# uc-vision/smart-tree

Hardware: AMD Instinct MI355X
Metric: points/sec end-to-end (voxelize->sparse-UNet->skeleton), 1M-pt tree (higher is better)
Workload: dtype f32

## Files before the change

### include/smarttree_hip.h

```cpp
#ifndef SMARTTREE_HIP_H
#define SMARTTREE_HIP_H

#include <stdint.h>

#ifdef __cplusplus
extern "C" {
#endif

int st_version(void);
#define ST_BRICK_NEED_COUNTS 4
#define ST_SKELETON_STATS_ENTRIES 16
#define ST_SKELETON_TUNING_ENTRIES 24
int st_abi_entries(int what);
const char* st_last_error(void);
int64_t st_query_workspace(int op, int64_t a, int64_t b, int64_t c);

int64_t st_scan_workspace_bytes(int64_t n);
int st_scan_u32(const uint32_t* in, uint32_t* out, int64_t n, uint32_t* total, void* ws, int64_t ws_bytes, void* stream);
int64_t st_sort_workspace_bytes(int64_t n);
int st_sort_pairs_u32(uint32_t* keys, uint32_t* vals, int64_t n, int key_bits, void* ws, int64_t ws_bytes, void* stream);

int64_t st_voxelize_workspace_bytes(int64_t n_points, int max_blocks, int64_t max_voxels);
int st_voxelize_blocks(const float* xyz, const float* rgb, int64_t n, double voxel_size, double block_size,
                       double buffer_size, int min_points, int max_blocks, int64_t max_voxels, float* feats,
                       int32_t* coords, uint8_t* mask, int64_t* point_index, float* block_centres,
                       int64_t* n_voxels_host, int64_t* n_blocks_host, void* ws, int64_t ws_bytes, void* stream);

int64_t st_hash_capacity(int64_t n);
int st_build_coord_hash(const int32_t* coords, int64_t n, unsigned long long* keys, unsigned* vals, int64_t cap, void* stream);
int st_build_subm_rulebook(const int32_t* coords, int64_t n, const unsigned long long* keys, const unsigned* vals,
                           int64_t cap, int32_t* nbr , void* stream);
int64_t st_spatial_order_workspace_bytes(int64_t n);
int st_spatial_order(const int32_t* coords, int64_t n, int32_t* order , void* ws, int64_t ws_bytes, void* stream);
int st_move_rows(const void* src, int row_words, const int32_t* order, int64_t n, void* dst, int scatter, void* stream);
int st_move_rows_list(const void* src, int row_words, const int32_t* order, const int32_t* list, int64_t n, void* dst, int scatter,
                      void* stream);
int64_t st_strided_workspace_bytes(int64_t n_fine);
int st_build_strided_outputs(const int32_t* coords, int64_t n, int64_t max_out, int32_t* out_coords,
                             unsigned long long* ckeys, unsigned* cvals, int64_t ccap, int64_t* n_out_host,
                             int32_t* extent_host , void* ws, int64_t ws_bytes, void* stream);
int st_build_strided_rulebook(const int32_t* coords, int64_t n, const unsigned long long* fkeys, const unsigned* fvals,
                              int64_t fcap, const int32_t* out_coords, int64_t n_out, const unsigned long long* ckeys,
                              const unsigned* cvals, int64_t ccap, const int32_t* extent_host,
                              int32_t* nbr_down , int32_t* nbr_up ,
                              int32_t* up_order ,
                              void* stream);

int st_sparse_conv_fwd(const float* x0, int c0, const float* x1, int cin, const int32_t* nbr, int K, int64_t n_out,
                       const float* w, int cout, const float* scale, const float* shift, const float* residual,
                       int relu, float* y, const int32_t* row_order ,
                       void* stream, int64_t nbr_stride );
int st_sparse_conv_mfma_fwd(const float* x0, int c0, const float* x1, int cin, const int32_t* nbr, int K, int64_t n_out,
                            const float* wp, int cout, const float* scale, const float* shift, const float* residual,
                            int relu, float* y, const int32_t* row_order ,
                            void* stream, int64_t nbr_stride ,
                            int variant );
int st_sparse_conv_b3_fwd(const float* x0, int c0, const float* x1, int cin, const int32_t* nbr, int K, int64_t n_out, const void* wq,
                          int cout, const float* scale, const float* shift, const float* residual, int relu, float* y,
                          const int32_t* row_order, void* stream, int64_t nbr_stride, int variant);
int st_sparse_conv_f16_fwd(const void* x0, int c0, const void* x1, int cin, const int32_t* nbr, int K, int64_t n_out,
                           const void* w, int cout, const float* scale, const float* shift, const void* residual, int relu,
                           void* y, int in_half, int out_half, const int32_t* row_order, void* stream, int64_t nbr_stride );
int st_sparse_conv_mfma_list_fwd(const float* x0, int c0, const float* x1, int cin, const int32_t* nbr, int K, int64_t n_out,
                                 const float* wp, int cout, const float* scale, const float* shift, const float* residual, int relu,
                                 float* y, const int32_t* row_order, void* stream, int64_t nbr_stride, int variant, int64_t level_rows,
                                 int parity);
int st_sparse_conv_b3_list_fwd(const float* x0, int c0, const float* x1, int cin, const int32_t* nbr, int K, int64_t n_out, const void* wq,
                               int cout, const float* scale, const float* shift, const float* residual, int relu, float* y,
                               const int32_t* row_order, void* stream, int64_t nbr_stride, int variant, int64_t level_rows, int parity);
int st_sparse_conv_f16_list_fwd(const void* x0, int c0, const void* x1, int cin, const int32_t* nbr, int K, int64_t n_out,
                                const void* w, int cout, const float* scale, const float* shift, const void* residual, int relu,
                                void* y, int in_half, int out_half, const int32_t* row_order, void* stream, int64_t nbr_stride,
                                int64_t level_rows, int parity);

int64_t st_brick_pyramid_workspace_bytes(int64_t n0, int n_blocks, int coord_bound, int depth, const int64_t* caps);
int st_brick_pyramid(const int32_t* coords0 , int64_t n0, int n_blocks ,
                     int coord_bound , int depth, const int32_t* blk_seg ,
                     int nseg, const int64_t* caps ,
                     int32_t* order0 , int32_t* const* coords_out ,
                     int32_t* const* subm , int32_t* const* down ,
                     int32_t* const* up , int32_t* const* up_order ,
                     int64_t* counts_host , void* ws, int64_t ws_bytes, void* stream);
int st_brick_pyramid_need(const int32_t* coords0, int64_t n0, int n_blocks, int coord_bound, int depth, const int32_t* blk_seg, int nseg,
                          const int64_t* caps, int32_t* order0, int32_t* const* coords_out, int32_t* const* subm, int32_t* const* down,
                          int32_t* const* up, int32_t* const* up_order, int64_t* counts_host, const unsigned char* inner ,
                          int32_t* const* need_order , int32_t* const* up_need ,
                          int64_t* need_counts_host , void* ws, int64_t ws_bytes, void* stream);
int st_head_param_floats(void);
int st_pointwise_mlp_heads(const float* x, int64_t n, const float* params, float* radius, float* direction,
                           float* class_l, float* medial_vector , int64_t* class_idx , void* stream);
int st_pointwise_mlp_heads_keep(const float* x, int64_t n, const unsigned char* keep, const float* params, float* radius, float* direction,
                                float* class_l, float* medial_vector , int64_t* class_idx , void* stream);

int st_centre_cloud(const float* xyz, int64_t n, float* out, void* ws, int64_t ws_bytes, void* stream);
int st_medial_points(const float* xyz, const float* mv, int64_t n, float* medial, float* radius, void* stream);
int64_t st_knn_workspace_bytes(int64_t n_dst);
int st_knn_radius(const float* src, int64_t n1, const float* dst, int64_t n2, int K, float r, const float* bound,
                  int bound_mode, float cell_hint, int64_t* idx, float* dist, void* ws, int64_t ws_bytes, void* stream);
int64_t st_make_edges_workspace_bytes(int64_t n);
int st_make_edges(const int64_t* idx, const float* dist, int64_t n, int K, int64_t* edges, float* w,
                  int64_t* n_edges_host, void* ws, int64_t ws_bytes, void* stream);
int64_t st_connected_components_workspace_bytes(int64_t n);
int st_connected_components(const int64_t* edges, int64_t E, int64_t n, int32_t* labels, void* ws, int64_t ws_bytes, void* stream);
int64_t st_component_layout_workspace_bytes(int64_t n);
int st_component_layout(const int32_t* labels, int64_t n, int min_vertices, int32_t* comp_size, int32_t* comp_off,
                        int32_t* vert_order, int32_t* new_id, int64_t* n_comp_host, int64_t* n_kept_host, void* ws,
                        int64_t ws_bytes, void* stream);
int64_t st_component_csr_workspace_bytes(int64_t m);
int st_component_csr(const int64_t* edges, const float* w, int64_t E, const int32_t* new_id, int64_t m, uint32_t* row_off,
                     uint32_t* col, float* wgt, void* ws, int64_t ws_bytes, void* stream);
int64_t st_skeleton_workspace_bytes(int64_t m, int64_t n_comp);
int st_skeleton_components(int n_comp, const int32_t* comp_off, const int32_t* comp_size_host, int64_t m, const float* pts,
                           const float* rad, const float* ysurf, const uint32_t* row_off, const uint32_t* col,
                           const float* wgt, float grid_cell, int stages, int block_threads, float* dist, int32_t* pred,
                           int32_t* root_local, float* tree_dist, int32_t* branch_parent, int32_t* branch_off,
                           int32_t* branch_len, int32_t* n_branches, int32_t* path_verts, int32_t* branch_of,
                           int64_t* stats_host, void* ws, int64_t ws_bytes, void* stream);
#define ST_SKELETON_STAGE_ARGS                                                                                          \
    int n_comp, const int32_t *comp_off, const int32_t *comp_size_host, int64_t m, const float *pts, const float *rad, \
        const float *ysurf, const uint32_t *row_off, const uint32_t *col, const float *wgt, float grid_cell,           \
        int block_threads, float *dist, int32_t *pred, int32_t *root_local, float *tree_dist, int32_t *branch_parent,  \
        int32_t *branch_off, int32_t *branch_len, int32_t *n_branches, int32_t *path_verts, int32_t *branch_of,        \
        int64_t *stats_host, void *ws, int64_t ws_bytes, void *stream
int st_sssp(ST_SKELETON_STAGE_ARGS);
int st_tree_distance(ST_SKELETON_STAGE_ARGS);
int st_sample_tree(ST_SKELETON_STAGE_ARGS);
int64_t st_assemble_workspace_bytes(int64_t cap_b);
int st_assemble_branches(int n_comp, const int32_t* comp_off, const int32_t* n_branches, const int32_t* branch_parent,
                         const int32_t* branch_off, const int32_t* branch_len, const int32_t* path_verts,
                         const int32_t* vert_order, const float* medial, const float* radius, int32_t* tree_off,
                         int32_t* parent, int32_t* start, int32_t* length, float* xyz, float* rad, int64_t cap_b,
                         int64_t cap_p, int64_t* counts_host, void* ws, int64_t ws_bytes, void* stream);
int st_post_process(int n_trees, const int32_t* tree_off, const int32_t* parent, const int32_t* start, const int32_t* len,
                    float* xyz, const float* rad_in, float* rad_out, uint8_t* keep, uint8_t* repaired, uint8_t* smoothed,
                    int32_t* depth_scratch, int do_prune, float min_radius, float min_length, int do_repair, int do_smooth, int kernel_size,
                    void* stream);

int st_points_to_nearest_tube(const float* pts, int64_t n, const float* a, const float* b, const float* r1, const float* r2,
                              int64_t m, float* vec, int64_t* idx, float* rad, void* stream);

int64_t st_sample_tubes_workspace_bytes(int64_t m);
int st_sample_tubes_count(const float* a, const float* b, int64_t m, double spacing, int32_t* count, int32_t* off,
                          int64_t* total_host, void* ws, int64_t ws_bytes, void* stream);
int st_sample_tubes_fill(const float* a, const float* b, const float* r1, const float* r2, int64_t m, double spacing,
                         const int32_t* off, int64_t total, float* pts, float* rad, int32_t* tube_of, void* stream);
int64_t st_skeleton_match_workspace_bytes(int64_t n);
int st_skeleton_match(const float* pts, const float* rad, int64_t n, const float* a, const float* b, const float* r1,
                      const float* r2, int64_t m, const float* thr, int n_thr, int ref_mode, float* dist, int32_t* idx,
                      float* tube_rad, void* tally, void* ws, int64_t ws_bytes, void* stream);

int st_centre_cloud_seg(const float* xyz, int64_t n, const int32_t* seg_off, int nseg, float* out, void* ws,
                        int64_t ws_bytes , void* stream);
int st_centre_cloud_box_seg(const float* xyz, int64_t n, const int32_t* seg_off, int nseg, float* out, void* ws,
                            int64_t ws_bytes , void* stream, float* box_out);
int st_voxelize_blocks_box_seg(const float* xyz, const float* rgb, int64_t n, const int32_t* seg_off, int nseg,
                               double voxel_size, double block_size, double buffer_size, int min_points, int max_blocks,
// ... 163 lines not shown
```

### smart_tree_amd/csrc/sparse_conv.hip

```cpp
#include "st_common.h"
#include "st_rule.h"

#define CONV_BLOCK 256

typedef _Float16 st_h;
typedef _Float16 st_v4h __attribute__((ext_vector_type(4)));
__device__ __forceinline__ float4 conv_load4(const float* p) { return *reinterpret_cast<const float4*>(p); }
__device__ __forceinline__ float4 conv_load4(const st_h* p) {
    const st_v4h v = *reinterpret_cast<const st_v4h*>(p);
    return make_float4((float)v.x, (float)v.y, (float)v.z, (float)v.w);
}
__device__ __forceinline__ void conv_store4(float* p, float a, float b, float c, float d) { *reinterpret_cast<float4*>(p) = make_float4(a, b, c, d); }
__device__ __forceinline__ void conv_store4(st_h* p, float a, float b, float c, float d) {
    *reinterpret_cast<st_v4h*>(p) = st_v4h{(st_h)a, (st_h)b, (st_h)c, (st_h)d};
}

template <int CIN, int COT, class TIN = float, class TOUT = float>
__global__ void __launch_bounds__(CONV_BLOCK) k_sparse_conv(const TIN* __restrict__ x0, int c0,
                                                            const TIN* __restrict__ x1, const int32_t* __restrict__ nbr,
                                                            int K, int64_t n_out, int64_t nstride, const float* __restrict__ w, int cout,
                                                            const float* __restrict__ scale, const float* __restrict__ shift,
                                                            const float* __restrict__ residual, int relu,
                                                            TOUT* __restrict__ y, const int32_t* __restrict__ row_order) {
    const int co_tiles = cout / COT;
    const int co0 = (int)(blockIdx.x % co_tiles) * COT;
    const int64_t pos = (int64_t)(blockIdx.x / co_tiles) * CONV_BLOCK + threadIdx.x;
    const bool active = pos < n_out;
    const int32_t entry = active && row_order ? row_order[pos] : 0;
    const int64_t o = active && row_order ? (int64_t)st_rule_row(entry) : pos;
    const uint32_t live = st_rule_live_offsets(entry, K);
    const int c1 = CIN - c0;
    float acc[COT];
#pragma unroll
    for (int c = 0; c < COT; c++) acc[c] = 0.0f;

    if (CIN % 4 == 0 && CIN <= 16) {
        constexpr int G = CIN <= 8 ? 9 : 3, Q = CIN / 4;
        for (int k0 = 0; k0 < K; k0 += G) {
            int idx[G];
            float4 v[G][Q];
#pragma unroll
            for (int j = 0; j < G; j++) {
                const int k = k0 + j;
                idx[j] = -1;
                if (k < K && active && ((live >> k) & 1u)) idx[j] = nbr ? nbr[(int64_t)k * nstride + o] : (int)o;
            }
#pragma unroll
            for (int j = 0; j < G; j++)
                if (idx[j] >= 0) {
#pragma unroll
                    for (int q = 0; q < Q; q++) {
                        const int ci = 4 * q;
                        const TIN* row = ci < c0 ? x0 + (int64_t)idx[j] * c0 + ci : x1 + (int64_t)idx[j] * c1 + (ci - c0);
                        v[j][q] = conv_load4(row);
                    }
                }
#pragma unroll
            for (int j = 0; j < G; j++) {
                if (idx[j] < 0) continue;
                const float* __restrict__ wk = w + (int64_t)(k0 + j) * CIN * cout + co0;
#pragma unroll
                for (int q = 0; q < Q; q++) {
                    const float xs[4] = {v[j][q].x, v[j][q].y, v[j][q].z, v[j][q].w};
#pragma unroll
                    for (int jj = 0; jj < 4; jj++)
#pragma unroll
                        for (int c = 0; c < COT; c++) acc[c] = fmaf(xs[jj], wk[(4 * q + jj) * cout + c], acc[c]);
                }
            }
        }
    } else
    for (int k = 0; k < K; k++) {
        int idx = -1;
        if (active && ((live >> k) & 1u)) idx = nbr ? nbr[(int64_t)k * nstride + o] : (int)o;
        if (idx < 0) continue;
        const float* __restrict__ wk = w + (int64_t)k * CIN * cout + co0;
        if (CIN % 4 == 0) {
#pragma unroll 2
            for (int ci = 0; ci < CIN; ci += 4) {
                const TIN* row = ci < c0 ? x0 + (int64_t)idx * c0 + ci : x1 + (int64_t)idx * c1 + (ci - c0);
                const float4 v = conv_load4(row);
                const float xs[4] = {v.x, v.y, v.z, v.w};
#pragma unroll
                for (int j = 0; j < 4; j++)
#pragma unroll
                    for (int c = 0; c < COT; c++) acc[c] = fmaf(xs[j], wk[(ci + j) * cout + c], acc[c]);
            }
        } else {
            for (int ci = 0; ci < CIN; ci++) {
                const float xv = (float)x0[(int64_t)idx * CIN + ci];
#pragma unroll
                for (int c = 0; c < COT; c++) acc[c] = fmaf(xv, wk[ci * cout + c], acc[c]);
            }
        }
    }
    if (!active) return;
#pragma unroll
    for (int c = 0; c < COT; c++) {
        float v = acc[c];
        if (scale) v = fmaf(v, scale[co0 + c], shift[co0 + c]);
        if (residual) v += residual[o * cout + co0 + c];
        if (relu) v = v > 0.0f ? v : 0.0f;
        acc[c] = v;
    }
    TOUT* out = y + o * cout + co0;
    if (COT % 4 == 0) {
#pragma unroll
        for (int c = 0; c < COT; c += 4) conv_store4(out + c, acc[c], acc[c + 1], acc[c + 2], acc[c + 3]);
    } else {
#pragma unroll
        for (int c = 0; c < COT; c++) out[c] = (TOUT)acc[c];
    }
}

__global__ void __launch_bounds__(CONV_BLOCK) k_sparse_conv_any(const float* __restrict__ x0, int c0, const float* __restrict__ x1, int cin,
                                                                const int32_t* __restrict__ nbr, int K, int64_t n_out, int64_t nstride,
                                                                const float* __restrict__ w, int cout, const float* __restrict__ scale,
                                                                const float* __restrict__ shift, const float* __restrict__ residual, int relu,
                                                                float* __restrict__ y, const int32_t* __restrict__ row_order) {
    const int64_t pos = (int64_t)blockIdx.x * CONV_BLOCK + threadIdx.x;
    if (pos >= n_out) return;
    const int co0 = (int)blockIdx.y * 4, nco = cout - co0 < 4 ? cout - co0 : 4;
    const int32_t entry = row_order ? row_order[pos] : 0;
    const int64_t o = row_order ? (int64_t)st_rule_row(entry) : pos;
    const uint32_t live = st_rule_live_offsets(entry, K);
    const int c1 = cin - c0;
    float acc[4] = {0.0f, 0.0f, 0.0f, 0.0f};
    for (int k = 0; k < K; k++) {
        if (K <= 32 && !((live >> k) & 1u)) continue;
        const int idx = nbr ? nbr[(int64_t)k * nstride + o] : (int)o;
        if (idx < 0) continue;
        const float* __restrict__ wk = w + (int64_t)k * cin * cout + co0;
        for (int ci = 0; ci < cin; ci++) {
            const float xv = ci < c0 ? x0[(int64_t)idx * c0 + ci] : x1[(int64_t)idx * c1 + (ci - c0)];
            for (int c = 0; c < nco; c++) acc[c] = fmaf(xv, wk[(int64_t)ci * cout + c], acc[c]);
        }
    }
    for (int c = 0; c < nco; c++) {
        float v = acc[c];
        if (scale) v = fmaf(v, scale[co0 + c], shift[co0 + c]);
        if (residual) v += residual[o * cout + co0 + c];
        if (relu) v = v > 0.0f ? v : 0.0f;
        y[o * cout + co0 + c] = v;
    }
}

struct ConvArgs {
    const void* x0;
    int c0;
    const void* x1;
    const int32_t* nbr;
    int K;
    int64_t n_out, nstride;
    const void* w;
    const float *scale, *shift;
    const void* residual;
    int relu;
    void* y;
    const int32_t* row_order;
    hipStream_t stream;
    int64_t level_rows = 0;
    bool parity = false;
};

static int conv_check_args(ConvArgs* a, int cin) {
    if (a->nstride <= 0) a->nstride = a->n_out;
    if (a->level_rows <= 0) { a->level_rows = a->n_out; a->parity = a->row_order != nullptr; }
    ST_REQUIRE(a->level_rows >= a->n_out && (a->level_rows == a->n_out || a->row_order != nullptr), "conv: a launch over fewer rows than the level has needs their list");
    ST_REQUIRE(a->K >= 1 && (a->nbr != nullptr || a->K == 1), "conv: a NULL neighbour table means pointwise (K = 1)");
    ST_REQUIRE(a->c0 > 0 && a->c0 <= cin && (a->c0 == cin || a->x1 != nullptr), "conv: bad concat split");
    ST_REQUIRE((a->scale == nullptr) == (a->shift == nullptr), "conv: scale and shift go together");
    return ST_OK;
}

template <int CIN, int COT, class TIN = float, class TOUT = float>
static int conv_launch(const ConvArgs& a, int cout) {
    int64_t blocks = st_div_up(a.n_out, CONV_BLOCK) * (cout / COT);
    hipLaunchKernelGGL((k_sparse_conv<CIN, COT, TIN, TOUT>), dim3((unsigned)blocks), dim3(CONV_BLOCK), 0, a.stream, (const TIN*)a.x0, a.c0,
                       (const TIN*)a.x1, a.nbr, a.K, a.n_out, a.nstride, (const float*)a.w, cout, a.scale, a.shift, (const float*)a.residual,
                       a.relu, (TOUT*)a.y, a.row_order);
    ST_CHECK_LAUNCH();
    return ST_OK;
}

typedef float st_v4f __attribute__((ext_vector_type(4)));
#define MF_BLOCK 256

struct MfF32 {
    typedef float T;
    typedef float4 W, A, B;
    static constexpr int CHUNK = 16, PLANES = 1;
    typedef float4 Row;
    static __device__ __forceinline__ Row no_row() { return make_float4(0.0f, 0.0f, 0.0f, 0.0f); }
    static __device__ __forceinline__ Row load_row(const T* row) { return *reinterpret_cast<const float4*>(row); }
    static __device__ __forceinline__ A fragment(const Row& r) { return r; }
    static __device__ __forceinline__ B load_b(const W* wc, int) { return *wc; }
    static __device__ __forceinline__ void mma(const A& a, const B& b, st_v4f& d) {
        d = __builtin_amdgcn_mfma_f32_16x16x4f32(a.x, b.x, d, 0, 0, 0);
        d = __builtin_amdgcn_mfma_f32_16x16x4f32(a.y, b.y, d, 0, 0, 0);
        d = __builtin_amdgcn_mfma_f32_16x16x4f32(a.z, b.z, d, 0, 0, 0);
        d = __builtin_amdgcn_mfma_f32_16x16x4f32(a.w, b.w, d, 0, 0, 0);
    }
};

typedef __bf16 st_bf8 __attribute__((ext_vector_type(8)));
struct StB3 { uint4 h, m, l; };
__device__ __forceinline__ unsigned b3_pack_hi(unsigned u0, unsigned u1) { return __builtin_amdgcn_perm(u1, u0, 0x07060302u); }
__device__ __forceinline__ void b3_split_pair(float a0, float a1, unsigned* h, unsigned* m, unsigned* l) {
    const unsigned u0 = __float_as_uint(a0), u1 = __float_as_uint(a1);
    *h = b3_pack_hi(u0, u1);
    const float r0 = a0 - __uint_as_float(u0 & 0xffff0000u), r1 = a1 - __uint_as_float(u1 & 0xffff0000u);
    const unsigned v0 = __float_as_uint(r0), v1 = __float_as_uint(r1);
    *m = b3_pack_hi(v0, v1);
    const float s0 = r0 - __uint_as_float(v0 & 0xffff0000u), s1 = r1 - __uint_as_float(v1 & 0xffff0000u);
    *l = b3_pack_hi(__float_as_uint(s0), __float_as_uint(s1));
}
__device__ __forceinline__ StB3 b3_split8(float4 a, float4 b) {
    StB3 o;
    b3_split_pair(a.x, a.y, &o.h.x, &o.m.x, &o.l.x);
    b3_split_pair(a.z, a.w, &o.h.y, &o.m.y, &o.l.y);
    b3_split_pair(b.x, b.y, &o.h.z, &o.m.z, &o.l.z);
    b3_split_pair(b.z, b.w, &o.h.w, &o.m.w, &o.l.w);
    return o;
}
__device__ __forceinline__ st_bf8 b3_bf8(uint4 v) { return __builtin_bit_cast(st_bf8, v); }

struct MfB3 {
    typedef float T;
    typedef uint4 W;
    typedef StB3 A;
    struct B { st_bf8 h, m, l; };
    static constexpr int CHUNK = 32, PLANES = 3;
    struct Row { float4 lo4, hi4; };
    static __device__ __forceinline__ Row no_row() { return Row{make_float4(0.0f, 0.0f, 0.0f, 0.0f), make_float4(0.0f, 0.0f, 0.0f, 0.0f)}; }
    static __device__ __forceinline__ Row load_row(const T* row) { return Row{*reinterpret_cast<const float4*>(row), *reinterpret_cast<const float4*>(row + 4)}; }
    static __device__ __forceinline__ A fragment(const Row& r) { return b3_split8(r.lo4, r.hi4); }
    static __device__ __forceinline__ B load_b(const W* wc, int plane) { return B{b3_bf8(wc[0]), b3_bf8(wc[plane]), b3_bf8(wc[2 * plane])}; }
    static __device__ __forceinline__ void mma(const A& a, const B& b, st_v4f& d) {
        const st_bf8 ah = b3_bf8(a.h), am = b3_bf8(a.m), al = b3_bf8(a.l);
        d = __builtin_amdgcn_mfma_f32_16x16x32_bf16(al, b.h, d, 0, 0, 0);
        d = __builtin_amdgcn_mfma_f32_16x16x32_bf16(ah, b.l, d, 0, 0, 0);
        d = __builtin_amdgcn_mfma_f32_16x16x32_bf16(am, b.m, d, 0, 0, 0);
        d = __builtin_amdgcn_mfma_f32_16x16x32_bf16(am, b.h, d, 0, 0, 0);
        d = __builtin_amdgcn_mfma_f32_16x16x32_bf16(ah, b.m, d, 0, 0, 0);
        d = __builtin_amdgcn_mfma_f32_16x16x32_bf16(ah, b.h, d, 0, 0, 0);
    }
};

typedef _Float16 st_v8h __attribute__((ext_vector_type(8)));
struct MfF16 {
    typedef st_h T;
    typedef st_v8h W, A, B;
    static constexpr int CHUNK = 32, PLANES = 1;
    typedef st_v8h Row;
    static __device__ __forceinline__ Row no_row() { return Row{}; }
    static __device__ __forceinline__ Row load_row(const T* row) { return *reinterpret_cast<const st_v8h*>(row); }
    static __device__ __forceinline__ A fragment(const Row& r) { return r; }
    static __device__ __forceinline__ B load_b(const W* wc, int) { return *wc; }
    static __device__ __forceinline__ void mma(const A& a, const B& b, st_v4f& d) { d = __builtin_amdgcn_mfma_f32_16x16x32_f16(a, b, d, 0, 0, 0); }
};

#define MF_PARAMS(T, W)                                                                                                               \
    const T *__restrict__ x0, int c0, const T *__restrict__ x1, const int32_t *__restrict__ nbr, int K, int64_t n_out, int64_t nstride, \
        const W *__restrict__ w, const float *__restrict__ scale, const float *__restrict__ shift, const T *__restrict__ residual,     \
        int relu, T *__restrict__ y, const int32_t *__restrict__ row_order
#define MF_ARGS x0, c0, x1, nbr, K, n_out, nstride, w, scale, shift, residual, relu, y, row_order

template <class OP, int CIN, int COUT, int RT, bool LDSW>
__device__ __forceinline__ void conv_rule_gemm(MF_PARAMS(typename OP::T, typename OP::W)) {
    typedef typename OP::T T;
    typedef typename OP::W W;
    constexpr bool PAIR = CIN == 16 && OP::CHUNK == 32;
    constexpr int CT = COUT / 16, NC = PAIR ? 1 : CIN / OP::CHUNK, LCH = OP::CHUNK / 4;
    constexpr int PLANE = 4 * COUT, WSTEP = NC * OP::PLANES * PLANE;
    __shared__ W wl[LDSW ? WSTEP : 1];
    const int tid = threadIdx.x, lane = tid & 63, wave = tid >> 6;
    const int i16 = lane & 15, g = lane >> 4;
    const int64_t obase = ((int64_t)blockIdx.x * (MF_BLOCK / 64) + wave) * (16 * RT);
    const int c1 = CIN - c0;
    st_v4f acc[RT][CT];
#pragma unroll
    for (int t = 0; t < RT; t++)
#pragma unroll
        for (int ct = 0; ct < CT; ct++) acc[t][ct] = st_v4f{0.0f, 0.0f, 0.0f, 0.0f};

    int64_t orow[RT];
    uint32_t live[RT];
#pragma unroll
    for (int t = 0; t < RT; t++) {
        const int64_t pos = obase + t * 16 + i16;
        const int32_t entry = pos < n_out && row_order ? row_order[pos] : 0;
        orow[t] = pos < n_out ? (row_order ? (int64_t)st_rule_row(entry) : pos) : -1;
        live[t] = st_rule_live_offsets(entry, K);
    }
    for (int j = 0; (PAIR ? 2 * j : j) < K; j++) {
        const int k = PAIR ? 2 * j + (g >> 1) : j;
        if (LDSW) {
            __syncthreads();
            for (int i = tid; i < WSTEP; i += MF_BLOCK) wl[i] = w[(int64_t)j * WSTEP + i];
        }
        int idx[RT];
        bool any = false;
#pragma unroll
        for (int t = 0; t < RT; t++) {
            idx[t] = (!PAIR || k < K) && orow[t] >= 0 && ((live[t] >> k) & 1u) ? (nbr ? nbr[(int64_t)k * nstride + orow[t]] : (int)orow[t]) : -1;
            any = any || idx[t] >= 0;
        }
        if (LDSW) __syncthreads();
        if (__ballot(any) == 0ull) continue;
        const W* wb = LDSW ? wl : w + (int64_t)j * WSTEP;
#pragma unroll
        for (int c = 0; c < NC; c++) {
            const int ci = PAIR ? LCH * (g & 1) : OP::CHUNK * c + LCH * g;
            typename OP::A a[RT];
#pragma unroll
            for (int t = 0; t < RT; t++) {
                typename OP::Row r = OP::no_row();
                if (idx[t] >= 0) {
                    const T* row = PAIR ? x0 + (int64_t)idx[t] * CIN + ci : ci < c0 ? x0 + (int64_t)idx[t] * c0 + ci : x1 + (int64_t)idx[t] * c1 + (ci - c0);
                    r = OP::load_row(row);
                }
                a[t] = OP::fragment(r);
            }
#pragma unroll
            for (int ct = 0; ct < CT; ct++) {
                const typename OP::B b = OP::load_b(wb + (c * OP::PLANES * 4 + g) * COUT + ct * 16 + i16, PLANE);
#pragma unroll
                for (int t = 0; t < RT; t++) OP::mma(a[t], b, acc[t][ct]);
            }
        }
    }
#pragma unroll
    for (int ct = 0; ct < CT; ct++) {
        const int ch = ct * 16 + i16;
        const float sc = scale ? scale[ch] : 1.0f, sh = scale ? shift[ch] : 0.0f;
#pragma unroll
        for (int t = 0; t < RT; t++)
#pragma unroll
            for (int r = 0; r < 4; r++) {
                const int64_t pos = obase + t * 16 + g * 4 + r;
                if (pos >= n_out) continue;
                const int64_t o = row_order ? (int64_t)st_rule_row(row_order[pos]) : pos;
                float v = acc[t][ct][r];
                if (scale) v = fmaf(v, sc, sh);
                if (residual) v += (float)residual[o * COUT + ch];
                if (relu) v = v > 0.0f ? v : 0.0f;
                y[o * COUT + ch] = (T)v;
            }
    }
}

template <int CIN, int COUT, int RT, bool LDSW>
__global__ void __launch_bounds__(MF_BLOCK) k_sparse_conv_mfma(MF_PARAMS(float, float4)) { conv_rule_gemm<MfF32, CIN, COUT, RT, LDSW>(MF_ARGS); }
template <int CIN, int COUT, int RT>
__global__ void __launch_bounds__(MF_BLOCK) k_sparse_conv_mfma_b3(MF_PARAMS(float, uint4)) { conv_rule_gemm<MfB3, CIN, COUT, RT, false>(MF_ARGS); }
template <int COUT, int RT>
__global__ void __launch_bounds__(MF_BLOCK) k_sparse_conv_mfma_b3_c16(MF_PARAMS(float, uint4)) { conv_rule_gemm<MfB3, 16, COUT, RT, false>(MF_ARGS); }
template <int CIN, int COUT, int RT>
__global__ void __launch_bounds__(MF_BLOCK) k_sparse_conv_mfma_f16x(MF_PARAMS(st_h, st_v8h)) { conv_rule_gemm<MfF16, CIN, COUT, RT, false>(MF_ARGS); }
template <int COUT, int RT>
__global__ void __launch_bounds__(MF_BLOCK) k_sparse_conv_mfma_f16x_c16(MF_PARAMS(st_h, st_v8h)) { conv_rule_gemm<MfF16, 16, COUT, RT, false>(MF_ARGS); }

template <class T, class W>
using mf_kernel_t = void (*)(MF_PARAMS(T, W));
template <int CIN, int COUT, int RT>
static mf_kernel_t<float, uint4> b3_kernel() {
    if constexpr (CIN == 16) return k_sparse_conv_mfma_b3_c16<COUT, RT>;
    else return k_sparse_conv_mfma_b3<CIN, COUT, RT>;
}
template <int CIN, int COUT, int RT>
static mf_kernel_t<st_h, st_v8h> f16x_kernel() {
    if constexpr (CIN == 16) return k_sparse_conv_mfma_f16x_c16<COUT, RT>;
    else return k_sparse_conv_mfma_f16x<CIN, COUT, RT>;
}

template <class T, class W>
static int mf_launch(mf_kernel_t<T, W> kernel, int rt, const ConvArgs& a) {
    hipLaunchKernelGGL(kernel, dim3((unsigned)st_div_up(a.n_out, (MF_BLOCK / 64) * 16 * rt)), dim3(MF_BLOCK), 0, a.stream, (const T*)a.x0, a.c0,
                       (const T*)a.x1, a.nbr, a.K, a.n_out, a.nstride, (const W*)a.w, a.scale, a.shift, (const T*)a.residual, a.relu, (T*)a.y,
                       a.row_order);
    ST_CHECK_LAUNCH();
    return ST_OK;
}

static int conv_row_tiles(const ConvArgs& a) { return a.level_rows >= (!a.parity ? 56000 : 300000) ? 2 : 1; }

template <int CIN, int COUT>
static int conv_launch_mfma(const ConvArgs& a, int v) {
    if (v == 0) v = (!a.parity && a.level_rows >= 150000) ? 18 : 1;
    switch (v) {
        case 1: return mf_launch(k_sparse_conv_mfma<CIN, COUT, 1, false>, 1, a);
        case 2: return mf_launch(k_sparse_conv_mfma<CIN, COUT, 2, false>, 2, a);
        case 4: return mf_launch(k_sparse_conv_mfma<CIN, COUT, 4, false>, 4, a);
        case 17: return mf_launch(k_sparse_conv_mfma<CIN, COUT, 1, true>, 1, a);
        default: return mf_launch(k_sparse_conv_mfma<CIN, COUT, 2, true>, 2, a);
    }
}

extern "C" int st_sparse_conv_b3_list_fwd(const float* x0, int c0, const float* x1, int cin, const int32_t* nbr, int K, int64_t n_out,
                                          const void* wq, int cout, const float* scale, const float* shift, const float* residual,
                                          int relu, float* y, const int32_t* row_order, void* stream_, int64_t nbr_stride, int variant,
                                          int64_t level_rows, int parity) {
    ConvArgs a = {x0, c0, x1, nbr, K, n_out, nbr_stride, wq, scale, shift, residual, relu, y, row_order, (hipStream_t)stream_, level_rows, parity != 0};
    ST_TRY(conv_check_args(&a, cin));
    ST_REQUIRE((cin % 32 == 0 || (cin == 16 && c0 == cin)) && cout % 16 == 0 && c0 % 8 == 0,
               "conv(b3): Cin % 32 (or Cin = 16 without concat), Cout % 16 and a concat split % 8 are required");
    if (n_out <= 0) return ST_OK;
    const int rt = variant == 1 || variant == 2 ? variant : conv_row_tiles(a);
#define B3_CASE(CI, CO) \
    if (cin == CI && cout == CO) return rt == 2 ? mf_launch(b3_kernel<CI, CO, 2>(), 2, a) : mf_launch(b3_kernel<CI, CO, 1>(), 1, a);
    B3_CASE(16, 16)
    B3_CASE(16, 32)
    B3_CASE(32, 16)
    B3_CASE(32, 32)
    B3_CASE(32, 64)
    B3_CASE(64, 32)
    B3_CASE(64, 64)
#undef B3_CASE
    st_set_error("conv(b3): no kernel instance for cin=%d cout=%d", cin, cout);
    return ST_ERR_INVALID;
}
extern "C" int st_sparse_conv_b3_fwd(const float* x0, int c0, const float* x1, int cin, const int32_t* nbr, int K, int64_t n_out,
                                     const void* wq, int cout, const float* scale, const float* shift, const float* residual,
                                     int relu, float* y, const int32_t* row_order, void* stream_, int64_t nbr_stride, int variant) {
    return st_sparse_conv_b3_list_fwd(x0, c0, x1, cin, nbr, K, n_out, wq, cout, scale, shift, residual, relu, y, row_order, stream_, nbr_stride,
                                      variant, 0, 0);
}

extern "C" int st_sparse_conv_f16_list_fwd(const void* x0, int c0, const void* x1, int cin, const int32_t* nbr, int K, int64_t n_out,
                                           const void* w, int cout, const float* scale, const float* shift, const void* residual,
                                           int relu, void* y, int in_half, int out_half, const int32_t* row_order, void* stream_,
                                           int64_t nbr_stride, int64_t level_rows, int parity) {
    ConvArgs a = {x0, c0, x1, nbr, K, n_out, nbr_stride, w, scale, shift, residual, relu, y, row_order, (hipStream_t)stream_, level_rows, parity != 0};
    ST_TRY(conv_check_args(&a, cin));
    ST_REQUIRE(in_half || out_half, "conv(f16): neither side is half precision -- use st_sparse_conv_fwd");
    if (n_out <= 0) return ST_OK;
    if (in_half && out_half) {
        ST_REQUIRE(cin % 16 == 0 && cout % 16 == 0 && c0 % 16 == 0, "conv(f16): channels and concat split must be multiples of 16");
        const int rt = conv_row_tiles(a);
#define F16X_CASE(CI, CO) \
    if (cin == CI && cout == CO) return rt == 2 ? mf_launch(f16x_kernel<CI, CO, 2>(), 2, a) : mf_launch(f16x_kernel<CI, CO, 1>(), 1, a);
        F16X_CASE(16, 16)
        F16X_CASE(16, 32)
        F16X_CASE(32, 16)
        F16X_CASE(32, 32)
        F16X_CASE(32, 64)
        F16X_CASE(64, 32)
        F16X_CASE(64, 64)
#undef F16X_CASE
        st_set_error("conv(f16): no kernel instance for cin=%d cout=%d", cin, cout);
        return ST_ERR_INVALID;
    }
    ST_REQUIRE(residual == nullptr && c0 == cin, "conv(f16): the converting kernels take no residual and no concat");
    ST_REQUIRE(cin % 4 == 0 && cout % 4 == 0, "conv(f16): channels must be multiples of 4");
#define CAST_CASE(CI, CO, COT_) \
    if (cin == CI && cout == CO) return in_half ? conv_launch<CI, COT_, st_h, float>(a, cout) : conv_launch<CI, COT_, float, st_h>(a, cout);
    CAST_CASE(8, 16, 16)
    CAST_CASE(16, 8, 8)
    CAST_CASE(16, 32, 16)
    CAST_CASE(32, 16, 16)
#undef CAST_CASE
    st_set_error("conv(f16): no converting kernel instance for cin=%d cout=%d", cin, cout);
    return ST_ERR_INVALID;
}
extern "C" int st_sparse_conv_f16_fwd(const void* x0, int c0, const void* x1, int cin, const int32_t* nbr, int K, int64_t n_out,
                                      const void* w, int cout, const float* scale, const float* shift, const void* residual,
                                      int relu, void* y, int in_half, int out_half, const int32_t* row_order, void* stream_,
                                      int64_t nbr_stride) {
    return st_sparse_conv_f16_list_fwd(x0, c0, x1, cin, nbr, K, n_out, w, cout, scale, shift, residual, relu, y, in_half, out_half, row_order,
                                       stream_, nbr_stride, 0, 0);
}

extern "C" int st_sparse_conv_mfma_list_fwd(const float* x0, int c0, const float* x1, int cin, const int32_t* nbr, int K,
                                            int64_t n_out, const float* wp, int cout, const float* scale, const float* shift,
                                            const float* residual, int relu, float* y, const int32_t* row_order, void* stream_,
                                            int64_t nbr_stride, int variant, int64_t level_rows, int parity) {
    ConvArgs a = {x0, c0, x1, nbr, K, n_out, nbr_stride, wp, scale, shift, residual, relu, y, row_order, (hipStream_t)stream_, level_rows, parity != 0};
    ST_TRY(conv_check_args(&a, cin));
    ST_REQUIRE(cin % 16 == 0 && cout % 16 == 0 && c0 % 16 == 0, "conv(mfma): channels and concat split must be multiples of 16");
    if (n_out <= 0) return ST_OK;
#define MFMA_CASE(CI, CO) \
    if (cin == CI && cout == CO) return conv_launch_mfma<CI, CO>(a, variant);
    MFMA_CASE(16, 16)
    MFMA_CASE(16, 32)
    MFMA_CASE(32, 16)
    MFMA_CASE(32, 32)
    MFMA_CASE(32, 64)
    MFMA_CASE(64, 32)
    MFMA_CASE(64, 64)
#undef MFMA_CASE
    st_set_error("conv(mfma): no kernel instance for cin=%d cout=%d", cin, cout);
    return ST_ERR_INVALID;
}
extern "C" int st_sparse_conv_mfma_fwd(const float* x0, int c0, const float* x1, int cin, const int32_t* nbr, int K,
                                       int64_t n_out, const float* wp, int cout, const float* scale, const float* shift,
                                       const float* residual, int relu, float* y, const int32_t* row_order, void* stream_,
                                       int64_t nbr_stride, int variant) {
    return st_sparse_conv_mfma_list_fwd(x0, c0, x1, cin, nbr, K, n_out, wp, cout, scale, shift, residual, relu, y, row_order, stream_, nbr_stride,
                                        variant, 0, 0);
}

extern "C" int st_sparse_conv_fwd(const float* x0, int c0, const float* x1, int cin, const int32_t* nbr, int K,
                                  int64_t n_out, const float* w, int cout, const float* scale, const float* shift,
                                  const float* residual, int relu, float* y, const int32_t* row_order, void* stream_,
                                  int64_t nbr_stride) {
    ConvArgs a = {x0, c0, x1, nbr, K, n_out, nbr_stride, w, scale, shift, residual, relu, y, row_order, (hipStream_t)stream_};
    ST_TRY(conv_check_args(&a, cin));
    ST_REQUIRE(cout >= 1, "conv: cout must be positive");
    if (n_out <= 0) return ST_OK;
#define CONV_CASE(CI, CO, COT_) \
    if (cin == CI && cout == CO && (c0 == cin || (CI % 4 == 0 && c0 % 4 == 0))) return conv_launch<CI, COT_>(a, cout);
    CONV_CASE(3, 8, 8)
    CONV_CASE(8, 8, 8)
    CONV_CASE(8, 16, 16)
    CONV_CASE(16, 8, 8)
    CONV_CASE(16, 16, 16)
    CONV_CASE(16, 32, 16)
    CONV_CASE(32, 16, 16)
    CONV_CASE(32, 32, 16)
    CONV_CASE(32, 64, 16)
    CONV_CASE(64, 32, 16)
    CONV_CASE(64, 64, 16)
#undef CONV_CASE
    hipLaunchKernelGGL(k_sparse_conv_any, dim3((unsigned)st_div_up(n_out, CONV_BLOCK), (unsigned)st_div_up(cout, 4)), dim3(CONV_BLOCK), 0, a.stream, x0, c0,
// ... 93 lines not shown
```

Before: 968.8 million.

## Use 32-bit addressing in sparse conv kernels and pipeline weight loads

```diff
diff --git a/include/smarttree_hip.h b/include/smarttree_hip.h
--- a/include/smarttree_hip.h
+++ b/include/smarttree_hip.h
@@ -72,6 +72,8 @@
                                 const void* w, int cout, const float* scale, const float* shift, const void* residual, int relu,
                                 void* y, int in_half, int out_half, const int32_t* row_order, void* stream, int64_t nbr_stride,
                                 int64_t level_rows, int parity);
+void st_sparse_conv_force_addr64(int on);
+int st_sparse_conv_last_addr32(void);
 
 int64_t st_brick_pyramid_workspace_bytes(int64_t n0, int n_blocks, int coord_bound, int depth, const int64_t* caps);
 int st_brick_pyramid(const int32_t* coords0 , int64_t n0, int n_blocks ,
diff --git a/smart_tree_amd/csrc/sparse_conv.hip b/smart_tree_amd/csrc/sparse_conv.hip
--- a/smart_tree_amd/csrc/sparse_conv.hip
+++ b/smart_tree_amd/csrc/sparse_conv.hip
@@ -1,3 +1,5 @@
+#include <atomic>
+
 #include "st_common.h"
 #include "st_rule.h"
 
@@ -15,35 +17,49 @@
     *reinterpret_cast<st_v4h*>(p) = st_v4h{(st_h)a, (st_h)b, (st_h)c, (st_h)d};
 }
 
-template <int CIN, int COT, class TIN = float, class TOUT = float>
+template <bool A64> struct ConvOff { typedef uint32_t t; };
+template <> struct ConvOff<true> { typedef int64_t t; };
+template <class T> __device__ __forceinline__ T* conv_at(T* base, uint32_t off) { return (T*)((const char*)base + off * (uint32_t)sizeof(T)); }
+template <class T> __device__ __forceinline__ T* conv_at(T* base, int64_t off) { return base + off; }
+
+#if defined(__HIP_DEVICE_COMPILE__)
+#define CONV_SCHED_FENCE() __builtin_amdgcn_sched_barrier(0)
+#else
+#define CONV_SCHED_FENCE() ((void)0)
+#endif
+
+template <int CIN, int COT, class TIN = float, class TOUT = float, bool A64 = true>
 __global__ void __launch_bounds__(CONV_BLOCK) k_sparse_conv(const TIN* __restrict__ x0, int c0,
                                                             const TIN* __restrict__ x1, const int32_t* __restrict__ nbr,
                                                             int K, int64_t n_out, int64_t nstride, const float* __restrict__ w, int cout,
                                                             const float* __restrict__ scale, const float* __restrict__ shift,
-                                                            const float* __restrict__ residual, int relu,
-                                                            TOUT* __restrict__ y, const int32_t* __restrict__ row_order) {
+                                                            const float* __restrict__ residual, TOUT* __restrict__ y, int relu,
+                                                            const int32_t* __restrict__ row_order) {
+    typedef typename ConvOff<A64>::t O;
     const int co_tiles = cout / COT;
     const int co0 = (int)(blockIdx.x % co_tiles) * COT;
     const int64_t pos = (int64_t)(blockIdx.x / co_tiles) * CONV_BLOCK + threadIdx.x;
     const bool active = pos < n_out;
     const int32_t entry = active && row_order ? row_order[pos] : 0;
-    const int64_t o = active && row_order ? (int64_t)st_rule_row(entry) : pos;
+    const O o = active && row_order ? (O)st_rule_row(entry) : (O)pos;
     const uint32_t live = st_rule_live_offsets(entry, K);
     const int c1 = CIN - c0;
     float acc[COT];
 #pragma unroll
     for (int c = 0; c < COT; c++) acc[c] = 0.0f;
 
-    if (CIN % 4 == 0 && CIN <= 16) {
+    if constexpr (CIN % 4 == 0 && CIN <= 16) {
         constexpr int G = CIN <= 8 ? 9 : 3, Q = CIN / 4;
+        constexpr int WS = 16, D = 1;
+        constexpr int SCI = WS / COT, SPO = CIN / SCI, NS = G * SPO;
         for (int k0 = 0; k0 < K; k0 += G) {
             int idx[G];
             float4 v[G][Q];
 #pragma unroll
             for (int j = 0; j < G; j++) {
-                const int k = k0 + j;
+                const int k = __builtin_amdgcn_readfirstlane(k0 + j);
                 idx[j] = -1;
-                if (k < K && active && ((live >> k) & 1u)) idx[j] = nbr ? nbr[(int64_t)k * nstride + o] : (int)o;
+                if (k < K && active && ((live >> k) & 1u)) idx[j] = nbr ? *conv_at(nbr, (O)k * (O)nstride + o) : (int)o;
             }
 #pragma unroll
             for (int j = 0; j < G; j++)
@@ -51,34 +67,48 @@
 #pragma unroll
                     for (int q = 0; q < Q; q++) {
                         const int ci = 4 * q;
-                        const TIN* row = ci < c0 ? x0 + (int64_t)idx[j] * c0 + ci : x1 + (int64_t)idx[j] * c1 + (ci - c0);
+                        const TIN* row = ci < c0 ? conv_at(x0, (O)idx[j] * (O)c0 + (O)ci) : conv_at(x1, (O)idx[j] * (O)c1 + (O)(ci - c0));
                         v[j][q] = conv_load4(row);
                     }
                 }
-#pragma unroll
-            for (int j = 0; j < G; j++) {
-                if (idx[j] < 0) continue;
-                const float* __restrict__ wk = w + (int64_t)(k0 + j) * CIN * cout + co0;
-#pragma unroll
-                for (int q = 0; q < Q; q++) {
-                    const float xs[4] = {v[j][q].x, v[j][q].y, v[j][q].z, v[j][q].w};
-#pragma unroll
-                    for (int jj = 0; jj < 4; jj++)
-#pragma unroll
-                        for (int c = 0; c < COT; c++) acc[c] = fmaf(xs[jj], wk[(4 * q + jj) * cout + c], acc[c]);
+            float wb[D + 1][WS];
+            auto load_stage = [&](float* ws, int s) {
+                const int k = k0 + s / SPO < K ? k0 + s / SPO : K - 1;
+                const float* __restrict__ wk = w + ((int64_t)k * CIN + SCI * (s % SPO)) * cout + co0;
+#pragma unroll
+                for (int i = 0; i < SCI; i++)
+#pragma unroll
+                    for (int c = 0; c < COT; c++) ws[i * COT + c] = wk[i * cout + c];
+            };
+#pragma unroll
+            for (int s = 0; s < D; s++) load_stage(wb[s], s);
+#pragma unroll
+            for (int s = 0; s < NS; s++) {
+                if (s + D < NS) load_stage(wb[(s + D) % (D + 1)], s + D);
+                CONV_SCHED_FENCE();
+                const int j = s / SPO, cb = SCI * (s % SPO);
+                if (idx[j] >= 0) {
+                    const float4 vq = v[j][cb / 4];
+                    const float xs[4] = {vq.x, vq.y, vq.z, vq.w};
+                    const float* wc = wb[s % (D + 1)];
+#pragma unroll
+                    for (int i = 0; i < SCI; i++)
+#pragma unroll
+                        for (int c = 0; c < COT; c++) acc[c] = fmaf(xs[cb % 4 + i], wc[i * COT + c], acc[c]);
                 }
+                CONV_SCHED_FENCE();
             }
         }
     } else
     for (int k = 0; k < K; k++) {
         int idx = -1;
-        if (active && ((live >> k) & 1u)) idx = nbr ? nbr[(int64_t)k * nstride + o] : (int)o;
+        if (active && ((live >> k) & 1u)) idx = nbr ? *conv_at(nbr, (O)k * (O)nstride + o) : (int)o;
         if (idx < 0) continue;
         const float* __restrict__ wk = w + (int64_t)k * CIN * cout + co0;
         if (CIN % 4 == 0) {
 #pragma unroll 2
             for (int ci = 0; ci < CIN; ci += 4) {
-                const TIN* row = ci < c0 ? x0 + (int64_t)idx * c0 + ci : x1 + (int64_t)idx * c1 + (ci - c0);
+                const TIN* row = ci < c0 ? conv_at(x0, (O)idx * (O)c0 + (O)ci) : conv_at(x1, (O)idx * (O)c1 + (O)(ci - c0));
                 const float4 v = conv_load4(row);
                 const float xs[4] = {v.x, v.y, v.z, v.w};
 #pragma unroll
@@ -88,22 +118,23 @@
             }
         } else {
             for (int ci = 0; ci < CIN; ci++) {
-                const float xv = (float)x0[(int64_t)idx * CIN + ci];
+                const float xv = (float)*conv_at(x0, (O)idx * (O)CIN + (O)ci);
 #pragma unroll
                 for (int c = 0; c < COT; c++) acc[c] = fmaf(xv, wk[ci * cout + c], acc[c]);
             }
         }
     }
     if (!active) return;
+    const O orow = o * (O)cout + (O)co0;
 #pragma unroll
     for (int c = 0; c < COT; c++) {
         float v = acc[c];
         if (scale) v = fmaf(v, scale[co0 + c], shift[co0 + c]);
-        if (residual) v += residual[o * cout + co0 + c];
+        if (residual) v += *conv_at(residual, orow + (O)c);
         if (relu) v = v > 0.0f ? v : 0.0f;
         acc[c] = v;
     }
-    TOUT* out = y + o * cout + co0;
+    TOUT* out = conv_at(y, orow);
     if (COT % 4 == 0) {
 #pragma unroll
         for (int c = 0; c < COT; c += 4) conv_store4(out + c, acc[c], acc[c + 1], acc[c + 2], acc[c + 3]);
@@ -173,12 +204,46 @@
     return ST_OK;
 }
 
+static uint64_t conv_extent(const void* p) {
+#ifdef ST_HIPEMU
+    (void)p;
+    return 1;
+#else
+    hipDeviceptr_t base = nullptr;
+    size_t size = 0;
+    if (hipMemGetAddressRange(&base, &size, (hipDeviceptr_t)p) != hipSuccess) {
+        (void)hipGetLastError();
+        return 0;
+    }
+    return (uint64_t)size - (uint64_t)((const char*)p - (const char*)base);
+#endif
+}
+
+#define CONV_ADDR32_LIMIT ((uint64_t)1 << 31)
+static std::atomic<int> conv_force_addr64{0}, conv_last_addr32{-1};
+extern "C" void st_sparse_conv_force_addr64(int on) { conv_force_addr64.store(on, std::memory_order_relaxed); }
+extern "C" int st_sparse_conv_last_addr32(void) { return conv_last_addr32.load(std::memory_order_relaxed); }
+
+static bool conv_addr32(const ConvArgs& a) {
+    bool ok = conv_force_addr64.load(std::memory_order_relaxed) == 0;
+    ok = ok && (a.nbr == nullptr || (uint64_t)a.K * (uint64_t)a.nstride * sizeof(int32_t) < CONV_ADDR32_LIMIT);
+    const void* arrays[4] = {a.x0, a.x1, a.residual, a.y};
+    for (int i = 0; ok && i < 4; i++)
+        if (arrays[i]) {
+            const uint64_t e = conv_extent(arrays[i]);
+            ok = e != 0 && e < CONV_ADDR32_LIMIT;
+        }
+    conv_last_addr32.store(ok ? 1 : 0, std::memory_order_relaxed);
+    return ok;
+}
+
 template <int CIN, int COT, class TIN = float, class TOUT = float>
 static int conv_launch(const ConvArgs& a, int cout) {
     int64_t blocks = st_div_up(a.n_out, CONV_BLOCK) * (cout / COT);
-    hipLaunchKernelGGL((k_sparse_conv<CIN, COT, TIN, TOUT>), dim3((unsigned)blocks), dim3(CONV_BLOCK), 0, a.stream, (const TIN*)a.x0, a.c0,
+    auto kernel = conv_addr32(a) ? k_sparse_conv<CIN, COT, TIN, TOUT, false> : k_sparse_conv<CIN, COT, TIN, TOUT, true>;
+    hipLaunchKernelGGL(kernel, dim3((unsigned)blocks), dim3(CONV_BLOCK), 0, a.stream, (const TIN*)a.x0, a.c0,
                        (const TIN*)a.x1, a.nbr, a.K, a.n_out, a.nstride, (const float*)a.w, cout, a.scale, a.shift, (const float*)a.residual,
-                       a.relu, (TOUT*)a.y, a.row_order);
+                       (TOUT*)a.y, a.relu, a.row_order);
     ST_CHECK_LAUNCH();
     return ST_OK;
 }
@@ -266,10 +331,11 @@
         int relu, T *__restrict__ y, const int32_t *__restrict__ row_order
 #define MF_ARGS x0, c0, x1, nbr, K, n_out, nstride, w, scale, shift, residual, relu, y, row_order
 
-template <class OP, int CIN, int COUT, int RT, bool LDSW>
+template <class OP, int CIN, int COUT, int RT, bool LDSW, bool A64>
 __device__ __forceinline__ void conv_rule_gemm(MF_PARAMS(typename OP::T, typename OP::W)) {
     typedef typename OP::T T;
     typedef typename OP::W W;
+    typedef typename ConvOff<A64>::t O;
     constexpr bool PAIR = CIN == 16 && OP::CHUNK == 32;
     constexpr int CT = COUT / 16, NC = PAIR ? 1 : CIN / OP::CHUNK, LCH = OP::CHUNK / 4;
     constexpr int PLANE = 4 * COUT, WSTEP = NC * OP::PLANES * PLANE;
@@ -284,14 +350,14 @@
 #pragma unroll
         for (int ct = 0; ct < CT; ct++) acc[t][ct] = st_v4f{0.0f, 0.0f, 0.0f, 0.0f};
 
-    int64_t orow[RT];
+    O orow[RT];
     uint32_t live[RT];
 #pragma unroll
     for (int t = 0; t < RT; t++) {
         const int64_t pos = obase + t * 16 + i16;
         const int32_t entry = pos < n_out && row_order ? row_order[pos] : 0;
-        orow[t] = pos < n_out ? (row_order ? (int64_t)st_rule_row(entry) : pos) : -1;
-        live[t] = st_rule_live_offsets(entry, K);
+        orow[t] = pos < n_out && row_order ? (O)st_rule_row(entry) : (O)pos;
+        live[t] = pos < n_out ? st_rule_live_offsets(entry, K) : 0u;
     }
     for (int j = 0; (PAIR ? 2 * j : j) < K; j++) {
         const int k = PAIR ? 2 * j + (g >> 1) : j;
@@ -303,7 +369,7 @@
         bool any = false;
 #pragma unroll
         for (int t = 0; t < RT; t++) {
-            idx[t] = (!PAIR || k < K) && orow[t] >= 0 && ((live[t] >> k) & 1u) ? (nbr ? nbr[(int64_t)k * nstride + orow[t]] : (int)orow[t]) : -1;
+            idx[t] = (!PAIR || k < K) && ((live[t] >> k) & 1u) ? (nbr ? *conv_at(nbr, (O)k * (O)nstride + orow[t]) : (int)orow[t]) : -1;
             any = any || idx[t] >= 0;
         }
         if (LDSW) __syncthreads();
@@ -317,7 +383,9 @@
             for (int t = 0; t < RT; t++) {
                 typename OP::Row r = OP::no_row();
                 if (idx[t] >= 0) {
-                    const T* row = PAIR ? x0 + (int64_t)idx[t] * CIN + ci : ci < c0 ? x0 + (int64_t)idx[t] * c0 + ci : x1 + (int64_t)idx[t] * c1 + (ci - c0);
+                    const T* row = PAIR      ? conv_at(x0, (O)idx[t] * (O)CIN + (O)ci)
+                                   : ci < c0 ? conv_at(x0, (O)idx[t] * (O)c0 + (O)ci)
+                                             : conv_at(x1, (O)idx[t] * (O)c1 + (O)(ci - c0));
                     r = OP::load_row(row);
                 }
                 a[t] = OP::fragment(r);
@@ -340,42 +408,44 @@
             for (int r = 0; r < 4; r++) {
                 const int64_t pos = obase + t * 16 + g * 4 + r;
                 if (pos >= n_out) continue;
-                const int64_t o = row_order ? (int64_t)st_rule_row(row_order[pos]) : pos;
+                const O o = (row_order ? (O)st_rule_row(row_order[pos]) : (O)pos) * (O)COUT + (O)ch;
                 float v = acc[t][ct][r];
                 if (scale) v = fmaf(v, sc, sh);
-                if (residual) v += (float)residual[o * COUT + ch];
+                if (residual) v += (float)*conv_at(residual, o);
                 if (relu) v = v > 0.0f ? v : 0.0f;
-                y[o * COUT + ch] = (T)v;
+                *conv_at(y, o) = (T)v;
             }
     }
 }
 
-template <int CIN, int COUT, int RT, bool LDSW>
-__global__ void __launch_bounds__(MF_BLOCK) k_sparse_conv_mfma(MF_PARAMS(float, float4)) { conv_rule_gemm<MfF32, CIN, COUT, RT, LDSW>(MF_ARGS); }
-template <int CIN, int COUT, int RT>
-__global__ void __launch_bounds__(MF_BLOCK) k_sparse_conv_mfma_b3(MF_PARAMS(float, uint4)) { conv_rule_gemm<MfB3, CIN, COUT, RT, false>(MF_ARGS); }
-template <int COUT, int RT>
-__global__ void __launch_bounds__(MF_BLOCK) k_sparse_conv_mfma_b3_c16(MF_PARAMS(float, uint4)) { conv_rule_gemm<MfB3, 16, COUT, RT, false>(MF_ARGS); }
-template <int CIN, int COUT, int RT>
-__global__ void __launch_bounds__(MF_BLOCK) k_sparse_conv_mfma_f16x(MF_PARAMS(st_h, st_v8h)) { conv_rule_gemm<MfF16, CIN, COUT, RT, false>(MF_ARGS); }
-template <int COUT, int RT>
-__global__ void __launch_bounds__(MF_BLOCK) k_sparse_conv_mfma_f16x_c16(MF_PARAMS(st_h, st_v8h)) { conv_rule_gemm<MfF16, 16, COUT, RT, false>(MF_ARGS); }
+#define MF_MIN_WAVES 2
+template <int CIN, int COUT, int RT, bool LDSW, bool A64>
+__global__ void __launch_bounds__(MF_BLOCK, MF_MIN_WAVES) k_sparse_conv_mfma(MF_PARAMS(float, float4)) { conv_rule_gemm<MfF32, CIN, COUT, RT, LDSW, A64>(MF_ARGS); }
+template <int CIN, int COUT, int RT, bool A64>
+__global__ void __launch_bounds__(MF_BLOCK, MF_MIN_WAVES) k_sparse_conv_mfma_b3(MF_PARAMS(float, uint4)) { conv_rule_gemm<MfB3, CIN, COUT, RT, false, A64>(MF_ARGS); }
+template <int COUT, int RT, bool A64>
+__global__ void __launch_bounds__(MF_BLOCK, MF_MIN_WAVES) k_sparse_conv_mfma_b3_c16(MF_PARAMS(float, uint4)) { conv_rule_gemm<MfB3, 16, COUT, RT, false, A64>(MF_ARGS); }
+template <int CIN, int COUT, int RT, bool A64>
+__global__ void __launch_bounds__(MF_BLOCK, MF_MIN_WAVES) k_sparse_conv_mfma_f16x(MF_PARAMS(st_h, st_v8h)) { conv_rule_gemm<MfF16, CIN, COUT, RT, false, A64>(MF_ARGS); }
+template <int COUT, int RT, bool A64>
+__global__ void __launch_bounds__(MF_BLOCK, MF_MIN_WAVES) k_sparse_conv_mfma_f16x_c16(MF_PARAMS(st_h, st_v8h)) { conv_rule_gemm<MfF16, 16, COUT, RT, false, A64>(MF_ARGS); }
 
 template <class T, class W>
 using mf_kernel_t = void (*)(MF_PARAMS(T, W));
-template <int CIN, int COUT, int RT>
+template <int CIN, int COUT, int RT, bool A64>
 static mf_kernel_t<float, uint4> b3_kernel() {
-    if constexpr (CIN == 16) return k_sparse_conv_mfma_b3_c16<COUT, RT>;
-    else return k_sparse_conv_mfma_b3<CIN, COUT, RT>;
-}
-template <int CIN, int COUT, int RT>
+    if constexpr (CIN == 16) return k_sparse_conv_mfma_b3_c16<COUT, RT, A64>;
+    else return k_sparse_conv_mfma_b3<CIN, COUT, RT, A64>;
+}
+template <int CIN, int COUT, int RT, bool A64>
 static mf_kernel_t<st_h, st_v8h> f16x_kernel() {
-    if constexpr (CIN == 16) return k_sparse_conv_mfma_f16x_c16<COUT, RT>;
-    else return k_sparse_conv_mfma_f16x<CIN, COUT, RT>;
+    if constexpr (CIN == 16) return k_sparse_conv_mfma_f16x_c16<COUT, RT, A64>;
+    else return k_sparse_conv_mfma_f16x<CIN, COUT, RT, A64>;
 }
 
 template <class T, class W>
-static int mf_launch(mf_kernel_t<T, W> kernel, int rt, const ConvArgs& a) {
+static int mf_launch(mf_kernel_t<T, W> k32, mf_kernel_t<T, W> k64, int rt, const ConvArgs& a) {
+    const mf_kernel_t<T, W> kernel = conv_addr32(a) ? k32 : k64;
     hipLaunchKernelGGL(kernel, dim3((unsigned)st_div_up(a.n_out, (MF_BLOCK / 64) * 16 * rt)), dim3(MF_BLOCK), 0, a.stream, (const T*)a.x0, a.c0,
                        (const T*)a.x1, a.nbr, a.K, a.n_out, a.nstride, (const W*)a.w, a.scale, a.shift, (const T*)a.residual, a.relu, (T*)a.y,
                        a.row_order);
@@ -389,11 +459,11 @@
 static int conv_launch_mfma(const ConvArgs& a, int v) {
     if (v == 0) v = (!a.parity && a.level_rows >= 150000) ? 18 : 1;
     switch (v) {
-        case 1: return mf_launch(k_sparse_conv_mfma<CIN, COUT, 1, false>, 1, a);
-        case 2: return mf_launch(k_sparse_conv_mfma<CIN, COUT, 2, false>, 2, a);
-        case 4: return mf_launch(k_sparse_conv_mfma<CIN, COUT, 4, false>, 4, a);
-        case 17: return mf_launch(k_sparse_conv_mfma<CIN, COUT, 1, true>, 1, a);
-        default: return mf_launch(k_sparse_conv_mfma<CIN, COUT, 2, true>, 2, a);
+        case 1: return mf_launch(k_sparse_conv_mfma<CIN, COUT, 1, false, false>, k_sparse_conv_mfma<CIN, COUT, 1, false, true>, 1, a);
+        case 2: return mf_launch(k_sparse_conv_mfma<CIN, COUT, 2, false, false>, k_sparse_conv_mfma<CIN, COUT, 2, false, true>, 2, a);
+        case 4: return mf_launch(k_sparse_conv_mfma<CIN, COUT, 4, false, false>, k_sparse_conv_mfma<CIN, COUT, 4, false, true>, 4, a);
+        case 17: return mf_launch(k_sparse_conv_mfma<CIN, COUT, 1, true, false>, k_sparse_conv_mfma<CIN, COUT, 1, true, true>, 1, a);
+        default: return mf_launch(k_sparse_conv_mfma<CIN, COUT, 2, true, false>, k_sparse_conv_mfma<CIN, COUT, 2, true, true>, 2, a);
     }
 }
 
@@ -408,7 +478,7 @@
     if (n_out <= 0) return ST_OK;
     const int rt = variant == 1 || variant == 2 ? variant : conv_row_tiles(a);
 #define B3_CASE(CI, CO) \
-    if (cin == CI && cout == CO) return rt == 2 ? mf_launch(b3_kernel<CI, CO, 2>(), 2, a) : mf_launch(b3_kernel<CI, CO, 1>(), 1, a);
+    if (cin == CI && cout == CO) return rt == 2 ? mf_launch(b3_kernel<CI, CO, 2, false>(), b3_kernel<CI, CO, 2, true>(), 2, a) : mf_launch(b3_kernel<CI, CO, 1, false>(), b3_kernel<CI, CO, 1, true>(), 1, a);
     B3_CASE(16, 16)
     B3_CASE(16, 32)
     B3_CASE(32, 16)
@@ -439,7 +509,7 @@
         ST_REQUIRE(cin % 16 == 0 && cout % 16 == 0 && c0 % 16 == 0, "conv(f16): channels and concat split must be multiples of 16");
         const int rt = conv_row_tiles(a);
 #define F16X_CASE(CI, CO) \
-    if (cin == CI && cout == CO) return rt == 2 ? mf_launch(f16x_kernel<CI, CO, 2>(), 2, a) : mf_launch(f16x_kernel<CI, CO, 1>(), 1, a);
+    if (cin == CI && cout == CO) return rt == 2 ? mf_launch(f16x_kernel<CI, CO, 2, false>(), f16x_kernel<CI, CO, 2, true>(), 2, a) : mf_launch(f16x_kernel<CI, CO, 1, false>(), f16x_kernel<CI, CO, 1, true>(), 1, a);
         F16X_CASE(16, 16)
         F16X_CASE(16, 32)
         F16X_CASE(32, 16)
```

After: 976.5 million (median of 6 runs). No clear change (+0.8%).
